# rosielab/emojivoice

Measured on AMD Instinct MI355X. Metric: audio_seconds_per_second, higher is better.
Workload: dtype f32 (deep layers: operand = two block-scaled fp16 pieces, product = 3 fp16 products on the fp16 MFMA, f32 accumulate); 1 GPU; config2: batch 64 x 516-frame (5.99 s) utterances per GPU, 10 Euler steps + HiFi-GAN V1, 22.05 kHz; global_batch=64, frames=516, ode_steps=10, parallelism=dp1, collective=none, batch_pipeline=cfm(i+1) || hifigan(i) on two streams, 2 pipeline(s) in flight

## Files before the change

### emojivoice_amd/_lib.py

```python
from __future__ import annotations

import ctypes as C
import os
import subprocess
from typing import Dict, Optional

import numpy as np
import torch

_HERE = os.path.dirname(os.path.abspath(__file__))
LIB_PATH = os.environ.get("EV_LIB_PATH") or os.path.join(_HERE, "lib", "libemojivoice_hip.so")
CSRC = os.path.join(_HERE, "csrc")
SOURCES = [os.path.join(CSRC, n) for n in ("ev_engine.hip", "ev_kernels.h", "ev_analysis_kernels.h", "ev_analysis.h")] \
    + [os.path.join(os.path.dirname(_HERE), "include", "emojivoice.h")]

EXPORTS = [
    "ev_abi_version", "ev_create", "ev_destroy", "ev_last_error", "ev_load_estimator", "ev_load_vocoder", "ev_load_vocoder_cfg", "ev_load_text_encoder", "ev_text_encoder",
    "ev_text_encoder_status", "ev_stft_magnitude", "ev_denoise", "ev_align", "ev_dbg_conv_bench",
    "ev_workspace_bytes", "ev_cfm_decode", "ev_estimator", "ev_hifigan", "ev_profile_enable", "ev_profile_read", "ev_profile_read_split", "ev_dbg_last_cfg", "ev_set_arithmetic", "ev_get_arithmetic",
    "ev_op_conv1d", "ev_op_groupnorm_mish", "ev_op_groupnorm_mish2", "ev_op_conv_groupnorm", "ev_op_layernorm", "ev_op_split_pieces", "ev_op_attention", "ev_op_ln_mlp", "ev_set_mrf_streams_max",
    "ev_cfm_decode2", "ev_reserve", "ev_alloc_count", "ev_dbg_sk_stats", "ev_op_attn_out", "ev_dbg_set_amax", "ev_dbg_set_attn_h16", "ev_dbg_set_chain", "ev_dbg_sk_taken",
    "ev_load_mel_basis", "ev_mel_spectrogram",
    "ev_maximum_path", "ev_log_prior", "ev_mas_align",
    "ev_estimator_rows", "ev_cfm_loss",
    "ev_load_resampler", "ev_resample", "ev_mel_stats",
    "ev_trim_bounds", "ev_trim_apply",
    "ev_pitch_yin", "ev_dtw",
    "ev_loudness",
    "ev_pyin_observe", "ev_pyin_decode",
    "ev_op_attention2", "ev_op_attn_out2",
    "ev_load_stoi", "ev_stoi",
    "ev_load_stft_dist", "ev_stft_dist",
    "ev_load_voice_quality", "ev_voice_quality",
    "ev_load_formants", "ev_formants",
    "ev_perturbation",
    "ev_load_harmonics", "ev_harmonics",
    "ev_functionals",
    "ev_load_auditory", "ev_auditory",
]


class EvLibraryError(RuntimeError):
    pass


class ev_tensor_index(C.Structure):
    _fields_ = [("name", C.c_char_p), ("offset", C.c_uint64), ("ndim", C.c_int32), ("shape", C.c_int64 * 4)]


class ev_model_dims(C.Structure):
    _fields_ = [("n_feats", C.c_int32), ("spk_emb_dim", C.c_int32), ("channels", C.c_int32), ("heads", C.c_int32),
                ("head_dim", C.c_int32)]


# ... 93 lines not shown
    lib.ev_trim_apply.argtypes = [vp, vp, vp, vp, f32, i32, i32, vp, i32, vp, vp]
    lib.ev_pitch_yin.argtypes = [vp, vp, vp, i32, i32, i32, i32, i32, i32, f32, vp, vp, vp, vp]
    lib.ev_dtw.argtypes = [vp, vp, vp, vp, vp, i32, i32, i32, i32, i32, vp, vp, vp, vp]
    lib.ev_loudness.argtypes = [vp, vp, vp, i32, i32, i32, vp, C.c_double, vp, vp, vp, vp, vp]
    f64 = C.c_double
    lib.ev_pyin_observe.argtypes = [vp, vp, vp, i32, i32, i32, i32, i32, i32, f64, f64, i32, i32, vp, i32, f64, f64, vp, vp, vp]
    lib.ev_pyin_decode.argtypes = [vp, vp, vp, vp, i32, i32, i32, i32, i32, vp, vp, f64, f64, vp, vp, vp, vp]
    lib.ev_load_stoi.argtypes = [vp, vp, vp, vp, i32, i32, i32, i32, i32]
    lib.ev_stoi.argtypes = [vp, vp, vp, vp, i32, i32, C.c_double, C.c_double, vp, vp, vp, vp, vp, vp]
    lib.ev_load_stft_dist.argtypes = [vp, vp, vp, i32, i32, i32]
    lib.ev_stft_dist.argtypes = [vp, vp, vp, vp, i32, i32, C.c_double, vp, vp, vp, vp]
    lib.ev_load_voice_quality.argtypes = [vp, vp, vp, i32, i32, i32, vp, vp, i32, i32, i32, vp, C.c_double]
    lib.ev_voice_quality.argtypes = [vp, vp, vp, i32, i32, C.c_double, vp, vp, vp, vp]
    lib.ev_load_formants.argtypes = [vp, vp, i32, i32, i32, C.c_double, C.c_double, C.c_double, i32]
    lib.ev_formants.argtypes = [vp, vp, vp, i32, i32, C.c_double, vp, vp, vp, vp]
    lib.ev_perturbation.argtypes = [vp, vp, vp, i32, i32, i32, vp, i32, i32, C.c_double, C.c_double, C.c_double, vp, vp, vp, vp]
    lib.ev_load_harmonics.argtypes = [vp, vp, vp, i32, i32, i32, C.c_double, i32, C.c_double, C.c_double, C.c_double]
    lib.ev_harmonics.argtypes = [vp, vp, vp, i32, i32, vp, vp, vp, i32, C.c_double, vp, vp, vp, vp]
    lib.ev_functionals.argtypes = [vp, vp, vp, vp, i32, i32, i32, vp, i32, vp, vp, vp]
    lib.ev_load_auditory.argtypes = [vp, vp, vp, i32, i32, i32, vp, i32, vp, vp, i32, i32, i32, C.c_double]
    lib.ev_auditory.argtypes = [vp, vp, vp, i32, i32, C.c_double, vp, vp, vp, vp, vp]
    lib.ev_maximum_path.argtypes = [vp, vp, vp, vp, i32, i32, i32, vp, vp, vp]
    lib.ev_log_prior.argtypes = [vp, vp, vp, i32, i32, i32, vp, vp]
    lib.ev_mas_align.argtypes = [vp, vp, vp, vp, vp, i32, i32, i32, vp, vp, vp, vp, vp]
    lib.ev_profile_enable.argtypes = [vp, i32]
    lib.ev_profile_read.argtypes = [vp, C.POINTER(C.c_double), C.POINTER(C.c_double), C.POINTER(C.c_int64), i32]
    lib.ev_profile_read_split.argtypes = [vp, C.POINTER(C.c_double), C.POINTER(C.c_double), C.POINTER(C.c_int64)]
    lib.ev_dbg_last_cfg.argtypes = [vp]
    lib.ev_set_arithmetic.argtypes = [vp, i32]
    lib.ev_get_arithmetic.argtypes = [vp]
    lib.ev_dbg_set_amax.argtypes = [vp, i32]
    lib.ev_dbg_set_attn_h16.argtypes = [vp, i32]
    lib.ev_dbg_set_chain.argtypes = [vp, i32]
    lib.ev_dbg_sk_taken.argtypes = [vp]
    lib.ev_dbg_sk_taken.restype = C.c_int64
    lib.ev_op_conv1d.argtypes = [vp, vp, vp, vp, i32, i32, i32, i32, i32, i32, i32, i32, i32, f32, vp, vp]
    lib.ev_op_groupnorm_mish.argtypes = [vp, vp, vp, vp, vp, i32, i32, i32, i32, vp, vp]
    lib.ev_op_groupnorm_mish2.argtypes = [vp, vp, vp, vp, vp, i32, i32, i32, i32, i32, vp, i32, vp, vp, vp]
    lib.ev_op_conv_groupnorm.argtypes = [vp, vp, vp, vp, i32, i32, i32, vp, vp, vp, i32, vp, vp, vp, vp, vp, C.POINTER(C.c_int), vp]
    lib.ev_op_layernorm.argtypes = [vp, vp, vp, vp, i32, i32, vp, vp]
    lib.ev_op_split_pieces.argtypes = [vp, vp, i32, vp, vp]
    lib.ev_op_attention.argtypes = [vp, vp, vp, i32, i32, i32, vp, vp]
    lib.ev_op_attn_out.argtypes = [vp, vp, vp, i32, i32, vp, vp, vp, vp]
    lib.ev_op_attention2.argtypes = [vp, vp, vp, i32, i32, i32, i32, i32, i32, vp, C.POINTER(C.c_int), vp]
    lib.ev_op_attn_out2.argtypes = [vp, vp, vp, i32, i32, i32, i32, vp, vp, f32, f32, f32, vp, C.POINTER(C.c_int), vp]
    lib.ev_op_ln_mlp.argtypes = [vp, vp, vp, vp, vp, vp, vp, vp, vp, vp, vp, i32, i32, i32, vp, vp]
    for n in EXPORTS:
        getattr(lib, n)
    _lib = lib
    return lib


def _stream_ptr() -> int:
    return int(torch.cuda.current_stream().cuda_stream)


def _ptr(t):
    return None if t is None else t.data_ptr()


class Engine:

    def __init__(self, device: int = 0, spk_emb_dim: int = 64, heads: int = 2):
        if not torch.cuda.is_available():
            raise EvLibraryError("no ROCm GPU visible: the EmojiVoice hot path has no CPU fallback")
        self.lib = load_library()
# ... 630 lines not shown
        assert F == 80
        wav = torch.empty((B, 1, T * 256), dtype=torch.float32, device=mel.device)
        per_utt = (T + 2 * self.voc_pad0) * self.voc_frame_bytes
        bmax = max(1, int((2**32 - 2**20) // per_utt))
        for b0 in range(0, B, bmax):
            b1 = min(B, b0 + bmax)
            self._check(self.lib.ev_hifigan(self.h, mel[b0:b1].data_ptr(), b1 - b0, T, wav[b0:b1].data_ptr(), _stream_ptr()), "ev_hifigan")
        return wav

    def workspace_bytes(self, B: int, Tp: int, Tv: int) -> int:
        return int(self.lib.ev_workspace_bytes(self.h, B, Tp, Tv))

    def profile_enable(self, on: bool):
        self._check(self.lib.ev_profile_enable(self.h, int(on)), "ev_profile_enable")

    def op_split_pieces(self, x):
        x = self._f32(x).reshape(-1)
        out = torch.empty((3, x.numel()), dtype=torch.float32, device=x.device)
        self._check(self.lib.ev_op_split_pieces(self.h, x.data_ptr(), x.numel(), out.data_ptr(), _stream_ptr()), "ev_op_split_pieces")
        return out

    def set_arithmetic(self, bf16_products: int):
        self._check(self.lib.ev_set_arithmetic(self.h, int(bf16_products)), "ev_set_arithmetic")

    def set_amax(self, on: bool) -> None:
        self._check(self.lib.ev_dbg_set_amax(self.h, int(bool(on))), "ev_dbg_set_amax")

    def set_attn_h16(self, on: bool) -> None:
        self._check(self.lib.ev_dbg_set_attn_h16(self.h, int(bool(on))), "ev_dbg_set_attn_h16")

    def set_chain(self, on: bool) -> None:
        self._check(self.lib.ev_dbg_set_chain(self.h, int(bool(on))), "ev_dbg_set_chain")

    def arithmetic(self) -> int:
        return int(self.lib.ev_get_arithmetic(self.h))

    def last_cfg(self) -> int:
        return int(self.lib.ev_dbg_last_cfg(self.h))

    def profile_read_split(self):
        ms, fl, n = C.c_double(), C.c_double(), C.c_int64()
        self._check(self.lib.ev_profile_read_split(self.h, C.byref(ms), C.byref(fl), C.byref(n)), "ev_profile_read_split")
        return ms.value, fl.value, n.value

    def profile_read(self, reset: bool = True):
        ms, fl, n = C.c_double(), C.c_double(), C.c_int64()
        self._check(self.lib.ev_profile_read(self.h, C.byref(ms), C.byref(fl), C.byref(n), int(reset)), "ev_profile_read")
        return ms.value, fl.value, n.value

    def op_conv1d(self, x, w, bias, dilation=1, transposed=False, stride=1, padding=0, pre_lrelu_slope=-1.0):
        x = self._f32(x)
        B, Cin, T = x.shape
        w = np.ascontiguousarray(w.detach().cpu().float().numpy())
        if transposed:
            Cout, K = w.shape[1], w.shape[2]
            Tout = T * stride
        else:
            Cout, K = w.shape[0], w.shape[2]
            Tout = T // stride
        bp = None
        if bias is not None:
            bnp = np.ascontiguousarray(bias.detach().cpu().float().numpy())
            bp = bnp.ctypes.data_as(C.c_void_p)
        y = torch.empty((B, Cout, Tout), dtype=torch.float32, device=x.device)
        self._check(self.lib.ev_op_conv1d(self.h, x.data_ptr(), w.ctypes.data_as(C.c_void_p), bp, B, Cin, T, Cout, K, dilation,
                                          int(transposed), stride, padding, float(pre_lrelu_slope), y.data_ptr(), _stream_ptr()),
# ... 129 lines not shown
```

### emojivoice_amd/csrc/ev_engine.hip

```cpp
#include "ev_kernels.h"
#include "../../include/emojivoice.h"

#include <math.h>
#include <stdlib.h>
#include <stdarg.h>
#include <stdio.h>
#include <string.h>

#include <algorithm>
#include <atomic>
#include <mutex>
#include <numeric>
#include <string>
#include <unordered_map>
#include <vector>

namespace {

struct HostTensor {
    const float* p = nullptr;
    int ndim = 0;
    int64_t shape[4] = {0, 0, 0, 0};
    int64_t numel() const { int64_t n = 1; for (int i = 0; i < ndim; ++i) n *= shape[i]; return n; }
};
// ... 89 lines not shown
    int device = 0;
    ev_model_dims dims;
    std::string err;
    std::vector<void*> owned;
    EstimatorW est;
    VocoderW voc;
    TextEncW enc;
    DenoiserW dn;
    MelBasisW melb;
    ResamplerW rs;
    StoiW stoi;
    StftDistW stftd;
    VoiceQW voiceq;
    FormantW fmt;
    HarmW harm;
    AudW aud;
    struct Scratch { char* p = nullptr; size_t bytes = 0; hipStream_t last = nullptr; bool last_valid = false; };
    Scratch dn_ws, enc_ws, mas_ws;
    Scratch dtw_ws;
    Scratch stat_ws;
    Scratch trim_ws;
    Scratch loud_ws;
    Scratch stoi_ws;
    Scratch stftd_ws;
    float* zeros = nullptr;
    int max_steps = 64;
    int* bad_ids_host = nullptr; int* bad_ids_dev = nullptr;
    char* ws = nullptr; size_t ws_bytes = 0; size_t ws_used = 0; size_t ws_bytes_last = 0;
    int ws_B = -1, ws_Tp = -1, ws_Tv = -1;
    bool prof = false;
    bool fuse_pairs = true;
    bool fuse_attn = true;
    bool attn_h16 = true;
    bool use_chain = true;
    bool fuse_mlp = true;
    int gn_stats_tiles = 0;
    int fuse_mlp_min_tiles = 96;
    std::vector<hipEvent_t> ev_pool; size_t ev_used = 0;
    hipStream_t ws_stream = nullptr; bool ws_stream_valid = false;
    float* temb_host[2] = {nullptr, nullptr}; size_t temb_cap[2] = {0, 0}; hipEvent_t temb_ev[2] = {nullptr, nullptr}; int temb_slot = 0;
    float* cap_pool = nullptr; size_t cap_stride = 0; int cap_used = 0; int cap_nt[8] = {0};
    struct TprojEntry { int nt; float* d; };
    std::vector<TprojEntry> tproj_cache;
    bool captured = false; int cap_B = 0, cap_Tp = 0;
    int64_t n_allocs = 0;
    double prof_flops = 0; int64_t prof_launches = 0;
    struct ProfRec { int kind, Cin, Cout, ntaps, nrows, cfg, lean; double flops; bool split = false; };
    std::vector<ProfRec> prof_recs;
    hipStream_t stream = nullptr;
    hipStream_t mrf_stream[2] = {nullptr, nullptr};
    hipEvent_t mrf_ev[4] = {nullptr, nullptr, nullptr, nullptr};
    int ncu = 0;
    unsigned* sk_ctrl = nullptr;
    unsigned sk_seq = 0;
    float* sk_part = nullptr;
    int split_terms = 16;
    bool use_amax = true;
    bool amax_emitted = false;
    int n_fp32_only_layers = 0;
    int last_cfg = -1;
    bool sk_balance = true;
    int sk_wgs = 2;
    int sk_spin = 3000;
    int mrf_max_frames = 16384;
    int force_cfg = -1;
    bool lean = true;
// ... 637 lines not shown
    p.X = X; p.ldx = C; p.Cin = C; p.isplit_log2 = 31;
    p.Mpad = Lc.Mpad; p.Kpad = Lc.Kpad;
    p.Y = Y; p.ldy = C; p.Cout = C; p.osplit_log2 = 31; p.mmul = 1;
    p.nrows = g.nrows; p.S = g.S; p.P = g.P; p.T = g.T;
    p.pro_lrelu = 1; p.pro_slope = 0.1f;
    p.scale = 1.f; p.ldr = C; p.accum = e.accum; p.div3 = e.div3; p.act2_lrelu = e.act2_lrelu; p.act2_slope = e.act2_slope;
    p.yold = e.yold; p.ymax_mul = 1; h->amax_emitted = false;
    p.mtiles = 1; p.ntiles = (g.nrows + out_rows - 1) / out_rows;
}
inline void resblock_bounds(ev_handle* h, ConvParams& p, const Epi& e) {
    if (e.ymax && (!e.accum || e.yold) && h->use_amax) { p.ymax = e.ymax; h->amax_emitted = true; }
}

int launch_pair(ev_handle* h, const ConvLayer& L1, const ConvLayer& L2, const float* X, float* Y, int C, const Geom& g, const Epi& e) {
    if (over_4gib(g, C)) return fail(h, "tensor exceeds the 4 GiB buffer-addressing limit: split the batch");
    if (L1.sparse_taps || L2.sparse_taps || L1.Kpad != C || L2.Kpad != C || L1.Kpad != L2.Kpad || L1.Mpad != L2.Mpad || L1.halo_lo != L1.halo_hi ||
        L2.halo_lo != L2.halo_hi || 2 * L2.halo_lo > 16 || !L1.bias || !L2.bias)
        return fail(h, "launch_pair: unsupported layer pair");
    if (C != 32 && C != 64 && C != 128) return fail(h, "launch_pair: C must be 32, 64 or 128");
    PairParams pp;
    memset(&pp, 0, sizeof pp);
    ConvParams& p = pp.c2;
    const int NT = 8192 / C;
    pp.h1 = L1.halo_lo; pp.h2 = L2.halo_lo; pp.mid_slope = 0.1f; pp.out_rows = NT - 2 * pp.h2;
    resblock_params(h, p, L2, X, Y, C, g, e, pp.out_rows);
    p.W = L2.W; p.bias = L2.bias; p.ntaps = L2.ntaps; p.taplist = L2.taplist[0];
    p.R = X;
    pp.W1 = L1.W; pp.W1x = L1.Wx; p.Wx = L2.Wx; pp.W1h = L1.Wh; pp.w1h_scale = L1.wh_scale; p.Wh = L2.Wh; p.wh_scale = L2.wh_scale; pp.b1 = L1.bias; pp.taplist1 = L1.taplist[0]; pp.ntaps1 = L1.ntaps;
    if (prof_begin(h)) return 1;
    const int lean = epi_flavour(p, h->lean);
    const int split_terms = h->split_terms;
    const bool split = split_terms > 0 && lean != 0 && L1.Wx && L2.Wx && !(e.force_cfg == 0);
    const bool h16 = split && split_terms == 16 && L1.Wh && L2.Wh;
    const dim3 grid(p.ntiles), block(256);
    dispatch<32, 64, 128>(C, [&](auto CC) {
        constexpr int WM = CC / 32, WN = 4 / WM;
        if (h16) {
            resblock_bounds(h, p, e);
            const size_t smem = std::max((size_t)(NT + EV_HALO) * (4 * C + 16) + 64, (size_t)4 * 32 * 36 * sizeof(float));
            dispatch<1, 3>(lean, [&](auto E) { launch<resblock_pair_h16_kernel<WM, WN, E>>(h->device, grid, block, smem, h->stream, pp); });
        } else if (split) {
            const size_t rsb = 6 * C + 16;
            const size_t xs = (size_t)(NT + ((2 * pp.h1 + 7) & ~7)) * rsb, ys = (size_t)(NT + 16) * rsb, es = (size_t)4 * 32 * 36 * sizeof(float);
            const size_t smem = std::max(xs, std::max(ys, es));
            dispatch<1, 3>(lean, [&](auto E) {
                dispatch<3, 6>(split_terms == 3 ? 3 : 6, [&](auto TT) { launch<resblock_pair_split_kernel<WM, WN, E, TT>>(h->device, grid, block, smem, h->stream, pp); });
            });
        } else {
            const size_t xs = (size_t)(NT + ((2 * pp.h1 + 7) & ~7)) * EV_LDK, ys = (size_t)(C / 32) * (NT + 16) * EV_LDK, es = (size_t)4 * 32 * 36;
            const size_t smem = std::max(xs, std::max(ys, es)) * sizeof(float);
            dispatch<0, 1, 3>(lean, [&](auto E) { launch<resblock_pair_kernel<WM, WN, E>>(h->device, grid, block, smem, h->stream, pp); });
        }
    });
    HIPCHK(h, hipGetLastError());
    const int code = (h16 ? 160 : split ? 140 : 100) + L2.ntaps;
    h->last_cfg = code;
    return h->prof ? prof_end(h, {1, C, C, L1.ntaps, g.nrows, code, lean, 2.0 * (L1.macs_per_row + L2.macs_per_row) * valid_rows(g), split}) : 0;
}

inline int chain_halo(const ConvLayer* L1, const ConvLayer* L2) { int hs = 0; for (int m = 0; m < 3; ++m) hs += L1[m].halo_lo + L2[m].halo_lo; return hs; }
inline bool chain_ok(const ev_handle* h, const ConvLayer* L1, const ConvLayer* L2, int C) {
    if (!h->use_chain || h->split_terms != 16 || (C != 32 && C != 64)) return false;
    int hb = 0;
    for (int m = 0; m < 3; ++m) {
        const ConvLayer &a = L1[m], &b = L2[m];
        if (!a.Wh || !b.Wh || !a.bias || !b.bias || a.sparse_taps || b.sparse_taps || a.Kpad != C || b.Kpad != C || a.Mpad != b.Mpad || a.Mpad != L1[0].Mpad ||
            a.halo_lo != a.halo_hi || b.halo_lo != b.halo_hi || a.ntaps != L1[0].ntaps || b.ntaps != L2[0].ntaps || a.ntaps > 64 || b.ntaps > 64) return false;
        hb = std::max(hb, std::max(a.halo_lo, b.halo_lo));
    }
    const int NT = C == 32 ? 256 : 128, hs = chain_halo(L1, L2);
    return hs <= 12 && 2 * hb <= EV_HALO && NT - 2 * hs >= NT / 2;
}
int launch_chain(ev_handle* h, const ConvLayer* L1, const ConvLayer* L2, const float* X, float* Y, int C, const Geom& g, const Epi& e) {
    if (over_4gib(g, C)) return fail(h, "tensor exceeds the 4 GiB buffer-addressing limit: split the batch");
    ChainParams cp;
    memset(&cp, 0, sizeof cp);
    ConvParams& p = cp.c2;
    int hb = 0;
    double macs = 0;
    for (int m = 0; m < 3; ++m) {
        cp.W1h[m] = L1[m].Wh; cp.W2h[m] = L2[m].Wh; cp.w1_scale[m] = L1[m].wh_scale; cp.w2_scale[m] = L2[m].wh_scale;
        cp.b1[m] = L1[m].bias; cp.b2[m] = L2[m].bias; cp.tl1[m] = L1[m].taplist[0]; cp.tl2[m] = L2[m].taplist[0];
        hb = std::max(hb, std::max(L1[m].halo_lo, L2[m].halo_lo));
        macs += L1[m].macs_per_row + L2[m].macs_per_row;
    }
    cp.ntaps1 = L1[0].ntaps; cp.ntaps2 = L2[0].ntaps; cp.hb = hb; cp.halo = chain_halo(L1, L2); cp.mid_slope = 0.1f;
    const int NT = 8192 / C;
    cp.out_rows = NT - 2 * cp.halo;
// ... 1811 lines not shown
            }
        }
    }
    if (conv_ms) *conv_ms = ms;
    if (conv_flops) *conv_flops = h->prof_flops;
    if (conv_launches) *conv_launches = h->prof_launches;
    if (reset) { h->ev_used = 0; h->prof_flops = 0; h->prof_launches = 0; h->prof_recs.clear(); }
    return 0;
}

int ev_dbg_last_cfg(ev_handle* h) { return h ? h->last_cfg : -1; }

int ev_set_arithmetic(ev_handle* h, int bf16_products) {
    if (!h) return 1;
    if (bf16_products != 0 && bf16_products != 3 && bf16_products != 6 && bf16_products != 9 && bf16_products != 16)
        return fail(h, "ev_set_arithmetic: 0, 3, 6, 9 or 16, got %d", bf16_products);
    h->split_terms = bf16_products;
    return 0;
}
int ev_get_arithmetic(ev_handle* h) { return h ? h->split_terms : -1; }

int ev_dbg_set_amax(ev_handle* h, int on) {
    if (!h) return 1;
    h->use_amax = on != 0;
    return 0;
}

int ev_dbg_set_chain(ev_handle* h, int on) {
    if (!h) return 1;
    h->use_chain = on != 0;
    return 0;
}

int ev_dbg_set_attn_h16(ev_handle* h, int on) {
    if (!h) return 1;
    h->attn_h16 = on != 0;
    return 0;
}

int ev_profile_read_split(ev_handle* h, double* ms_out, double* flops_out, int64_t* launches_out) {
    if (!h) return 1;
    HIPCHK(h, hipStreamSynchronize(h->stream));
    double ms = 0, fl = 0;
    int64_t n = 0;
    if (h->prof_recs.size() * 2 == h->ev_used)
        for (size_t i = 0; i < h->prof_recs.size(); ++i) {
            const auto& r = h->prof_recs[i];
            if (!r.split) continue;
            float t = 0;
            HIPCHK(h, hipEventElapsedTime(&t, h->ev_pool[2 * i], h->ev_pool[2 * i + 1]));
            ms += t; fl += r.flops; n += 1;
        }
    if (ms_out) *ms_out = ms;
    if (flops_out) *flops_out = fl;
    if (launches_out) *launches_out = n;
    return 0;
}

int ev_dbg_conv_bench(ev_handle* h, int Cin, int Cout, int K, int dil, int B, int T, int P, int iters, int dbg, int cfg, float* ms_out) {
    const int stagger = (dbg & 64) ? 0 : -1;
    const bool planar = (dbg & 32) != 0;
    const bool no_res = (dbg & 128) != 0;
    const bool no_pro = (dbg & 512) != 0;
    dbg &= ~(64 | 32 | 128 | 512);
    if (enter(h)) return 1;
    h->stream = nullptr;
// ... 384 lines not shown
```

### emojivoice_amd/csrc/ev_kernels.h

```cpp
#pragma once
#include <hip/hip_runtime.h>
#include <stdint.h>
#include <type_traits>

typedef float f32x16 __attribute__((ext_vector_type(16)));
typedef float f32x4 __attribute__((ext_vector_type(4)));
typedef int i32x4 __attribute__((ext_vector_type(4)));

#define EV_MAX_TAPS 16
#define EV_BK 32
#define EV_LDK 36
#define EV_WROWS 128
#define EV_SK_MAXF4(TW) ((TW) == 4 ? (64 + 64) * 8 * 8 : 16 * 512)
#define EV_HALO 64

enum { ACT_NONE = 0, ACT_LRELU = 1, ACT_TANH = 2, ACT_SILU = 3, ACT_MISH = 4, ACT_SNAKE = 5 };

struct SkCtl {
    unsigned* ctrl;
    unsigned* flags;
    float* part;
    int part_floats;
    int q, r;
    int spin_limit;
// ... 2381 lines not shown
    {
#pragma unroll
        for (int j = 0; j < TN; ++j) {
            const int r = wn * (TN * 32) + j * 32 + li;
            const int n = g0 + r;
            const int t = (n >= 0 && n < p.nrows) ? (n % p.S) - p.P : -1;
            const float inside = (t >= 0 && t < p.T) ? 1.f : 0.f;
#pragma unroll
            for (int g = 0; g < 4; ++g) {
                f32x4 v;
#pragma unroll
                for (int e = 0; e < 4; ++e) v[e] = ev_lrelu(acc[0][j][4 * g + e], pp.mid_slope) * inside;
                *(f32x4*)(Ys + (wm * YROWS + r + pp.h2) * EV_LDK + 8 * g + 4 * lh) = v;
            }
        }
        if (tid < 2 * pp.h2 * 8 * NCH) {
            const int chn = tid / (2 * pp.h2 * 8), rem = tid % (2 * pp.h2 * 8);
            const int br = rem / 8, c4 = (rem % 8) * 4;
            const int row = br < pp.h2 ? br : NT + br;
            f32x4 z = {0.f, 0.f, 0.f, 0.f};
            *(f32x4*)(Ys + (chn * YROWS + row) * EV_LDK + c4) = z;
        }
    }
    ev_lds_barrier();

    phase(p.W, p.taplist, p.ntaps, LEAN ? p.bias : nullptr, [&](int ch) -> const float* {
        return Ys + (ch * YROWS + wn * (TN * 32) + li + pp.h2) * EV_LDK + 4 * lh;
    });

    if constexpr (LEAN != 0) conv_epilogue_lean<TM, TN, LEAN>(p, acc, smem + wave * (32 * (TM * 32 + 4)), wm * 32, g0 + wn * (TN * 32), lane, n0, n0 + pp.out_rows);
    else conv_epilogue<TM, TN, false>(p, acc, smem + wave * (32 * (TM * 32 + 4)), wm * 32, g0 + wn * (TN * 32), lane, n0, n0 + pp.out_rows);
}

template <int WAVES_M, int WAVES_N, class PIPE>
struct EvResblockCore {
    static constexpr int TM = 1, TN = 2;
    static constexpr int C = 32 * WAVES_M;
    static constexpr int NT = WAVES_N * TN * 32;
    static constexpr int PIECES = PIPE::PIECES;
    static constexpr unsigned KGB = PIPE::KG_BYTES;
    static constexpr int RSB = PIECES * 2 * C + 16;
    static constexpr int NS = C / 16, H = NS / 2;
    static_assert(WAVES_M * WAVES_N == 4, "4 waves per workgroup");

    char* Xb;
    float* red;
    int tid, lane, wave, wm, wn, li, lh;
    unsigned wlane, wbase;
    f32x16 acc[TM][TN];
    f32x4 A0[PIECES][TM], A1[PIECES][TM], A2[PIECES][TM], A3[PIECES][TM], B0[PIECES][TN], B1[PIECES][TN];

    __device__ __forceinline__ EvResblockCore(char* tile, float* maxima, int Kpad) : Xb(tile), red(maxima) {
        tid = threadIdx.x; lane = tid & 63; wave = __builtin_amdgcn_readfirstlane(tid >> 6);
        wm = wave / WAVES_N; wn = wave % WAVES_N;
        li = lane & 31; lh = lane >> 5;
        wlane = (unsigned)lane * 16u;
        wbase = (unsigned)(wm * (Kpad >> 4)) * KGB;
    }
    __device__ __forceinline__ int row0() const { return wn * (TN * 32); }
    __device__ __forceinline__ const char* bbase(int halo) const { return Xb + (row0() + li + halo) * RSB + 16 * lh; }
    __device__ __forceinline__ bool row_inside(const ConvParams& p, int g0, int j) const {
        const int n = g0 + row0() + j * 32 + li;
        const int t = (n >= 0 && n < p.nrows) ? (n % p.S) - p.P : -1;
        return t >= 0 && t < p.T;
    }

    __device__ __forceinline__ void ldAp(const __amdgpu_buffer_rsrc_t& rW, f32x4 (&dst)[PIECES][TM], unsigned aoff) {
#pragma unroll
        for (int pc = 0; pc < PIECES; ++pc) dst[pc][0] = ev_bload4(rW, wlane, aoff + (unsigned)(pc * 1024));
    }
    __device__ __forceinline__ void ldB(f32x4 (&dst)[PIECES][TN], const char* brow, int slab) {
#pragma unroll
        for (int pc = 0; pc < PIECES; ++pc)
#pragma unroll
            for (int j = 0; j < TN; ++j) dst[pc][j] = *(const f32x4*)(brow + j * 32 * RSB + pc * (2 * C) + slab * 32);
    }
    __device__ __forceinline__ unsigned g_off(int2 tlv, int g, int ngroups) const {
        const int gg = g < ngroups ? g : 0;
        return PIPE::tap_off((unsigned)__builtin_amdgcn_readlane(tlv.x, gg / H)) + wbase + (unsigned)(2 * (gg % H)) * KGB;
    }
    __device__ __forceinline__ int g_row(int2 tlv, int g, int ngroups) const {
        const int gg = g < ngroups ? g : 0;
        return __builtin_amdgcn_readlane(tlv.y, gg / H);
    }
    __device__ __forceinline__ void acc_init(const float* binit, float unit) {
        f32x4 bq[4];
#pragma unroll
        for (int g = 0; g < 4; ++g) bq[g] = *(const f32x4*)(binit + wm * 32 + 8 * g + 4 * lh) * unit;
#pragma unroll
        for (int b = 0; b < TN; ++b)
#pragma unroll
            for (int r = 0; r < 16; ++r) acc[0][b][r] = bq[r >> 2][r & 3];
    }
    __device__ __forceinline__ void ring_fill(const __amdgpu_buffer_rsrc_t& rW, int2 tlv, int ngroups) {
        const unsigned o0 = g_off(tlv, 0, ngroups), o1 = g_off(tlv, 1, ngroups);
        ldAp(rW, A0, o0); ldAp(rW, A1, o0 + KGB); ldAp(rW, A2, o1); ldAp(rW, A3, o1 + KGB);
    }
    __device__ __forceinline__ void group(const __amdgpu_buffer_rsrc_t& rW, int2 tlv, int ngroups, const char* brow0,
                                          f32x4 (&Aa)[PIECES][TM], f32x4 (&Ab)[PIECES][TM], int g) {
        const char* brow = brow0 + g_row(tlv, g, ngroups) * RSB;
        const char* nbrow = brow0 + g_row(tlv, g + 1, ngroups) * RSB;
        const int s0 = 2 * (g % H), ns0 = 2 * ((g + 1) % H);
        const unsigned nap = g_off(tlv, g + 2, ngroups);
        ldB(B1, brow, s0 + 1);
        __builtin_amdgcn_sched_barrier(0);
        PIPE::template mma<TM, TN>(acc, Aa, B0);
        __builtin_amdgcn_sched_barrier(0);
        ldAp(rW, Aa, nap);
        ldB(B0, nbrow, ns0);
        __builtin_amdgcn_sched_barrier(0);
        PIPE::template mma<TM, TN>(acc, Ab, B1);
        __builtin_amdgcn_sched_barrier(0);
        ldAp(rW, Ab, nap + KGB);
    }
    __device__ __forceinline__ void kloop(const __amdgpu_buffer_rsrc_t& rW, int2 tlv, int ngroups, const char* brow0) {
        ldB(B0, brow0 + g_row(tlv, 0, ngroups) * RSB, 0);
        int g = 0;
        for (; g + 1 < ngroups; g += 2) { group(rW, tlv, ngroups, brow0, A0, A1, g); group(rW, tlv, ngroups, brow0, A2, A3, g + 1); }
        if (g < ngroups) group(rW, tlv, ngroups, brow0, A0, A1, g);
    }
    template <int ROW16>
    __device__ __forceinline__ void zero_border_rows(int hb) {
        for (int i = tid; i < 2 * hb * ROW16; i += 256) {
            const int br = i / ROW16, c16 = i % ROW16;
            const int row = br < hb ? br : NT + br;
            uint4 z = {0u, 0u, 0u, 0u};
            *(uint4*)(Xb + row * RSB + c16 * 16) = z;
        }
    }

    __device__ __forceinline__ float hand_over(f32x16 (&v)[TN], int slot, int row_halo) {
        float mx = 0.f;
#pragma unroll
        for (int j = 0; j < TN; ++j)
#pragma unroll
            for (int r = 0; r < 16; r += 2) mx = fmaxf(mx, fmaxf(fabsf(v[j][r]), fabsf(v[j][r + 1])));
        float tmx = evh_wg_max(red, slot, wave, lane, mx);
        if (!evh_is_finite(tmx)) {
            mx = 0.f;
#pragma unroll
            for (int j = 0; j < TN; ++j)
#pragma unroll
                for (int r = 0; r < 16; ++r) { const float a = fabsf(v[j][r]); mx = fmaxf(mx, evh_is_finite(a) ? a : 0.f); }
            tmx = evh_wg_max(red, 8 + slot, wave, lane, mx);
        }
        const float sc = evh_scale_for(tmx);
#pragma unroll
        for (int j = 0; j < TN; ++j) {
            const int r = row0() + j * 32 + li;
#pragma unroll
            for (int g = 0; g < 4; ++g) {
                const f32x4 w = {v[j][4 * g] * sc, v[j][4 * g + 1] * sc, v[j][4 * g + 2] * sc, v[j][4 * g + 3] * sc};
                uint2 q0v, q1v;
                evh_split4(w, q0v, q1v);
                char* dst = Xb + (r + row_halo) * RSB + (wm * 32 + 8 * g + 4 * lh) * 2;
                *(uint2*)(dst) = q0v; *(uint2*)(dst + 2 * C) = q1v;
            }
        }
        return sc;
    }
    __device__ __forceinline__ float conv_from_acc(int slot, int row_halo, const __amdgpu_buffer_rsrc_t& rW, int2 tlv, int ngroups,
                                                   const float* bias, float w_scale) {
        const float u = w_scale * hand_over(acc[0], slot, row_halo);
        acc_init(bias, u);
        ev_lds_barrier();
        kloop(rW, tlv, ngroups, bbase(row_halo));
        return u;
    }

    __device__ __forceinline__ void running_x_load(const ConvParams& p, int g0, int hb, f32x16 (&xr)[TN], float (&inside)[TN]) {
        const __amdgpu_buffer_rsrc_t rX = ev_rsrc(p.X);
#pragma unroll
        for (int j = 0; j < TN; ++j) {
            const int n = g0 + row0() + j * 32 + li;
            const bool in = n >= 0 && n < p.nrows;
            inside[j] = row_inside(p, g0, j) ? 1.f : 0.f;
            const unsigned ro = (in ? (unsigned)n * (unsigned)p.ldx : 0u) * 4u + (unsigned)(wm * 32 + 4 * lh) * 4u;
#pragma unroll
            for (int q = 0; q < 4; ++q) {
                const f32x4 v = ev_bload4(rX, ro + (unsigned)(8 * q) * 4u, 0);
#pragma unroll
                for (int e = 0; e < 4; ++e) xr[j][4 * q + e] = v[e];
            }
        }
        zero_border_rows<RSB / 16>(hb);
    }
    __device__ __forceinline__ void acc_from_lrelu_x(const f32x16 (&xr)[TN], float slope) {
#pragma unroll
        for (int j = 0; j < TN; ++j)
#pragma unroll
            for (int r = 0; r < 16; ++r) acc[0][j][r] = ev_lrelu(xr[j][r], slope);
    }
    __device__ __forceinline__ void running_x_add(f32x16 (&xr)[TN], const float (&inside)[TN], float u) {
        const float inv = 1.0f / u;
#pragma unroll
        for (int j = 0; j < TN; ++j)
#pragma unroll
            for (int r = 0; r < 16; ++r) xr[j][r] = fmaf(acc[0][j][r], inv, xr[j][r]) * inside[j];
    }
    template <int LEAN>
    __device__ __forceinline__ void running_x_store(const ConvParams& p, EvAmax& am, const f32x16 (&xr)[TN], float* smem, int g0, int n0, int out_rows) {
#pragma unroll
        for (int j = 0; j < TN; ++j) acc[0][j] = xr[j];
        ev_amax_from_acc<TM, TN>(p, am, acc, g0 + row0(), lane);
        conv_epilogue_lean<TM, TN, LEAN>(p, acc, smem + wave * (32 * (TM * 32 + 4)), wm * 32, g0 + row0(), lane, n0, n0 + out_rows);
        ev_amax_emit(p, am, g0 + row0(), TN * 32, lane);
    }
};
// ... 53 lines not shown
        }
    }
    ev_lds_barrier();
    k.kloop(rW1, tlv1, ng1, k.bbase(pp.h1));
    k.ring_fill(rW2, tlv2, ng2);

    ev_lds_barrier();
    {
#pragma unroll
        for (int j = 0; j < TN; ++j) {
            const int r = k.row0() + j * 32 + li;
            const float inside = k.row_inside(p, g0, j) ? 1.f : 0.f;
#pragma unroll
            for (int g = 0; g < 4; ++g) {
                f32x4 v;
#pragma unroll
                for (int e = 0; e < 4; ++e) v[e] = ev_lrelu(k.acc[0][j][4 * g + e], pp.mid_slope) * inside;
                uint2 q0v, q1v, q2v;
                evx_split4(v, q0v, q1v, q2v);
                char* dst = Xb + (r + pp.h2) * RSB + (wm * 32 + 8 * g + 4 * lh) * 2;
                *(uint2*)(dst) = q0v; *(uint2*)(dst + 2 * C) = q1v; *(uint2*)(dst + 4 * C) = q2v;
            }
        }
        k.template zero_border_rows<6 * C / 16>(pp.h2);
    }
    k.acc_init(LEAN ? p.bias : pp.b1, 1.f);
    ev_lds_barrier();

    k.kloop(rW2, tlv2, ng2, k.bbase(pp.h2));

    conv_epilogue_lean<TM, TN, LEAN>(p, k.acc, smem + wave * (32 * (TM * 32 + 4)), wm * 32, g0 + k.row0(), lane, n0, n0 + pp.out_rows);
}

template <int WAVES_M, int WAVES_N, int LEAN>
__global__ __launch_bounds__(256, 2) void resblock_pair_h16_kernel(const PairParams pp) {
    using Core = EvResblockCore<WAVES_M, WAVES_N, EvPipeH16>;
    constexpr int TM = Core::TM, TN = Core::TN, C = Core::C, NT = Core::NT, RSB = Core::RSB, H = Core::H;
    constexpr int TPR = C / 4, RPS = 256 / TPR;
    constexpr int XPASS = (NT + EV_HALO) / RPS;
    const ConvParams& p = pp.c2;
    extern __shared__ __attribute__((aligned(16))) float smem[];

    const int nt = ev_xcd_remap(blockIdx.x, p.ntiles);
    const int n0 = nt * pp.out_rows;
    const int g0 = n0 - pp.h2;
    if (ev_tile_is_padding(p.S, p.P, p.T, p.nrows, n0, pp.out_rows)) return;
    Core k((char*)smem, smem + ((NT + EV_HALO) * RSB) / 4, p.Kpad);
    char* Xb = k.Xb;
    const int tid = k.tid, lane = k.lane, wave = k.wave, wm = k.wm;
    const int srow = tid / TPR, sc4 = (tid % TPR) * 4;
    const int nw0 = g0 + k.row0();
    EvAmax am = ev_amax_begin(p, nw0, TN * 32);
    const __amdgpu_buffer_rsrc_t rX = ev_rsrc(p.X);

    const __amdgpu_buffer_rsrc_t rW1 = ev_rsrc(pp.W1h), rW2 = ev_rsrc(p.Wh);
    const int ng1 = pp.ntaps1 * H, ng2 = p.ntaps * H;
    const int2 tlv1 = (lane < pp.ntaps1) ? pp.taplist1[lane] : make_int2(0, 0);
    const int2 tlv2 = (lane < p.ntaps) ? p.taplist[lane] : make_int2(0, 0);
    k.ring_fill(rW1, tlv1, ng1);
    float sx;
    {
        const int xrows = NT + 2 * pp.h1;
        f32x4 xg[XPASS];
        float mx = 0.f;
#pragma unroll
        for (int q = 0; q < XPASS; ++q) {
            const int r = q * RPS + srow;
            const int gr = g0 - pp.h1 + r;
            xg[q] = ev_bload4(rX, ((r < xrows && gr >= 0 && gr < p.nrows) ? (unsigned)gr * (unsigned)p.ldx : 0u) * 4u + (unsigned)sc4 * 4u, 0);
        }
#pragma unroll
        for (int q = 0; q < XPASS; ++q) mx = fmaxf(mx, evh_absmax4(xg[q]));
        float tmx = evh_wg_max(k.red, 0, wave, lane, mx);
        if (!evh_is_finite(tmx)) {
            mx = 0.f;
#pragma unroll
            for (int q = 0; q < XPASS; ++q) mx = fmaxf(mx, evh_absmax4_finite(xg[q]));
            tmx = evh_wg_max(k.red, 8, wave, lane, mx);
        }
        sx = evh_scale_for(tmx);
        am.rlo = am.rhi = tmx;
#pragma unroll
        for (int q = 0; q < XPASS; ++q) {
            const int r = q * RPS + srow;
            f32x4 v = xg[q];
            v[0] = ev_lrelu(v[0], p.pro_slope); v[1] = ev_lrelu(v[1], p.pro_slope);
            v[2] = ev_lrelu(v[2], p.pro_slope); v[3] = ev_lrelu(v[3], p.pro_slope);
            uint2 q0v, q1v;
            evh_split4(v * sx, q0v, q1v);
            if (r < xrows) {
                char* dst = Xb + r * RSB + sc4 * 2;
                *(uint2*)(dst) = q0v; *(uint2*)(dst + 2 * C) = q1v;
            }
        }
    }
    const float u1 = pp.w1h_scale * sx;
    k.acc_init(pp.b1, u1);
    ev_lds_barrier();
    k.kloop(rW1, tlv1, ng1, k.bbase(pp.h1));
    k.ring_fill(rW2, tlv2, ng2);

    float sy;
    {
        const float inv1 = 1.0f / u1;
#pragma unroll
        for (int j = 0; j < TN; ++j) {
            const float inside = k.row_inside(p, g0, j) ? inv1 : 0.f;
#pragma unroll
            for (int r16 = 0; r16 < 16; ++r16) k.acc[0][j][r16] = ev_lrelu(k.acc[0][j][r16] * inside, pp.mid_slope);
        }
        sy = k.hand_over(k.acc[0], 4, pp.h2);
        k.template zero_border_rows<4 * C / 16>(pp.h2);
    }
    const float u2 = p.wh_scale * sy;
    k.acc_init(LEAN ? p.bias : pp.b1, u2);
    ev_lds_barrier();

    k.kloop(rW2, tlv2, ng2, k.bbase(pp.h2));
    {
        const float inv2 = 1.0f / u2;
#pragma unroll
        for (int j = 0; j < TN; ++j)
#pragma unroll
            for (int r16 = 0; r16 < 16; ++r16) k.acc[0][j][r16] *= inv2;
    }
    ev_amax_from_acc<TM, TN>(p, am, k.acc, nw0, lane);
    conv_epilogue_lean<TM, TN, LEAN>(p, k.acc, smem + wave * (32 * (TM * 32 + 4)), wm * 32, nw0, lane, n0, n0 + pp.out_rows);
    ev_amax_emit(p, am, nw0, TN * 32, lane);
}

struct ChainParams {
    ConvParams c2;
    const void* W1h[3]; const void* W2h[3]; float w1_scale[3], w2_scale[3];
    const float* b1[3]; const float* b2[3];
    const int2* tl1[3]; const int2* tl2[3];
    int ntaps1, ntaps2;
    int hb;
    int halo;
    int out_rows;
    float mid_slope;
};
template <int WAVES_M, int WAVES_N, int LEAN>
__global__ __launch_bounds__(256, 2) void resblock_chain_h16_kernel(const ChainParams cp) {
    using Core = EvResblockCore<WAVES_M, WAVES_N, EvPipeH16>;
    constexpr int TN = Core::TN, C = Core::C, NT = Core::NT, RSB = Core::RSB, H = Core::H;
    static_assert(C == 32 || C == 64, "C = 32 / 64");
    const ConvParams& p = cp.c2;
    extern __shared__ __attribute__((aligned(16))) float smem[];
    const int nt = ev_xcd_remap(blockIdx.x, p.ntiles);
    const int n0 = nt * cp.out_rows;
    const int g0 = n0 - cp.halo;
    if (ev_tile_is_padding(p.S, p.P, p.T, p.nrows, n0, cp.out_rows)) return;
    Core k((char*)smem, smem + ((NT + EV_HALO) * RSB) / 4, p.Kpad);
    const int lane = k.lane;
    EvAmax am = ev_amax_begin(p, g0 + k.row0(), TN * 32);
    f32x16 xr[TN];
    float inside[TN];
    k.running_x_load(p, g0, cp.hb, xr, inside);
    const int ng1 = cp.ntaps1 * H, ng2 = cp.ntaps2 * H;
#pragma unroll 1
    for (int m = 0; m < 3; ++m) {
        const __amdgpu_buffer_rsrc_t rW1 = ev_rsrc(cp.W1h[m]), rW2 = ev_rsrc(cp.W2h[m]);
// ... 2801 lines not shown
```

### include/emojivoice.h

```cpp
#ifndef EMOJIVOICE_H
#define EMOJIVOICE_H

#include <stddef.h>
#include <stdint.h>

#ifdef __cplusplus
extern "C" {
#endif

#define EV_ABI_VERSION 4

typedef struct ev_handle ev_handle;

typedef struct ev_tensor_index {
    const char *name;
    uint64_t offset;
    int32_t ndim;
    int64_t shape[4];
} ev_tensor_index;

typedef struct ev_model_dims {
    int32_t n_feats;
    int32_t spk_emb_dim;
    int32_t channels;
// ... 136 lines not shown
int ev_load_harmonics(ev_handle *h, const double *window , const double *twiddle , int W, int H, int nfft,
                      double sr, int n_harm, double search , double min_spacing , double a3_range );
int ev_harmonics(ev_handle *h, const float *d_x , const int32_t *d_len , int B, int L,
                 const float *d_period ,
                 const double *d_formant , const int32_t *d_fcount , int n_formants,
                 double power_floor, double *d_frame , int32_t *d_count ,
                 double *d_harm , void *stream);

int ev_functionals(ev_handle *h, const double *d_v , const uint8_t *d_mask ,
                   const int32_t *d_len , int B, int K, int F,
                   const double *q , int NQ,
                   double *d_stat , int32_t *d_count , void *stream);

int ev_load_auditory(ev_handle *h, const double *window , const double *twiddle , int W, int H, int nfft,
                     const double *mel_w , int n_mel, const double *eq ,
                     const double *dct , int n_ceps, int k_lo, int k_hi, double compress );
int ev_auditory(ev_handle *h, const float *d_x , const int32_t *d_len , int B, int L, double power_floor,
                double *d_frame , double *d_mfcc , int32_t *d_flags ,
                double *d_bands , void *stream);

int ev_profile_enable(ev_handle *h, int on);
int ev_profile_read(ev_handle *h, double *conv_ms, double *conv_flops, int64_t *conv_launches, int reset);
int ev_profile_read_split(ev_handle *h, double *ms, double *flops, int64_t *launches);
int ev_set_arithmetic(ev_handle *h, int setting);
int ev_get_arithmetic(ev_handle *h);

int ev_dbg_last_cfg(ev_handle *h);

int ev_dbg_conv_bench(ev_handle *h, int Cin, int Cout, int K, int dil, int B, int T, int P, int iters, int dbg, int cfg, float *ms_out);

int ev_dbg_set_amax(ev_handle *h, int on);
int ev_dbg_set_attn_h16(ev_handle *h, int on);
int ev_dbg_set_chain(ev_handle *h, int on);

int ev_dbg_sk_stats(ev_handle *h, uint32_t *out3);
int64_t ev_dbg_sk_taken(ev_handle *h);

int ev_op_conv1d(ev_handle *h, const float *d_x , const float *w ,
                 const float *bias , int B, int Cin, int T, int Cout, int K, int dilation,
                 int transposed, int stride, int padding, float pre_lrelu_slope , float *d_y, void *stream);
int ev_op_groupnorm_mish(ev_handle *h, const float *d_x , const float *d_gamma, const float *d_beta,
                         const int32_t *d_lengths, int B, int C, int T, int groups, float *d_y, void *stream);
int ev_op_groupnorm_mish2(ev_handle *h, const float *d_x , const float *d_gamma, const float *d_beta,
                          const int32_t *d_lengths, int B, int C, int T, int groups, int mode, const float *d_temb,
                          int temb_stride, const float *d_R, float *d_y, void *stream);
int ev_op_conv_groupnorm(ev_handle *h, const float *d_x , const float *w ,
                         const float *bias , int Cin, int T, int K, const float *d_gamma,
                         const float *d_beta, const int32_t *d_lengths , int mode, const float *d_temb, const float *d_R,
                         float *d_conv, float *d_part, float *d_y, int *tiles_out, void *stream);
int ev_op_split_pieces(ev_handle *h, const float *d_x, int n, float *d_pieces, void *stream);
int ev_op_layernorm(ev_handle *h, const float *d_x , const float *d_gamma, const float *d_beta, int rows,
                    int C, float *d_y, void *stream);
int ev_op_ln_mlp(ev_handle *h, const float *d_x, const float *d_ln_g, const float *d_ln_b, const float *w1, const float *b1,
                 const float *d_alpha_exp, const float *d_beta_inv, const float *w2, const float *b2, const float *d_rowmask,
                 int rows, int M1, int mode, float *d_y, void *stream);
int ev_op_attention(ev_handle *h, const float *d_qkv , const int32_t *d_lengths, int B, int T,
                    int heads, float *d_out , void *stream);

int ev_op_attn_out(ev_handle *h, const float *d_qkv, const int32_t *d_lengths, int B, int T, const float *w_out, const float *b_out,
                   float *d_hid, void *stream);

int ev_op_attention2(ev_handle *h, const float *d_qkv, const int32_t *d_lengths, int B, int S, int P, int T, int heads, int no_scratch,
                     float *d_out, int *ran, void *stream);
int ev_op_attn_out2(ev_handle *h, const float *d_qkv, const int32_t *d_lengths, int B, int S, int P, int T, const float *w_out,
                    const float *b_out, float sq, float sk, float sv, float *d_hid, int *ran, void *stream);

// ... 5 lines not shown
```

Before: 4822 audio_s/s.

## Add wide-row resblock pair kernel for 128-channel HiFi-GAN layers

Adds a resblock pair kernel variant where each wave computes two 32-channel tiles (TM=2) for C=128. The 2x2 wave layout doubles the row tile to 128 with a 16-row halo, so halo recompute and weight reloads per output row go down. It is selected only when there are enough tiles (at least 5 workgroups per CU) and the kernel taps are small. The cost is more registers and LDS per workgroup, which may lower occupancy. A debug knob sets the threshold and counts launches.

Result: no change. 4839 audio_s/s, median of 6 (+0.3%).

```diff
diff --git a/emojivoice_amd/_lib.py b/emojivoice_amd/_lib.py
--- a/emojivoice_amd/_lib.py
+++ b/emojivoice_amd/_lib.py
@@ -19,7 +19,7 @@
     "ev_text_encoder_status", "ev_stft_magnitude", "ev_denoise", "ev_align", "ev_dbg_conv_bench",
     "ev_workspace_bytes", "ev_cfm_decode", "ev_estimator", "ev_hifigan", "ev_profile_enable", "ev_profile_read", "ev_profile_read_split", "ev_dbg_last_cfg", "ev_set_arithmetic", "ev_get_arithmetic",
     "ev_op_conv1d", "ev_op_groupnorm_mish", "ev_op_groupnorm_mish2", "ev_op_conv_groupnorm", "ev_op_layernorm", "ev_op_split_pieces", "ev_op_attention", "ev_op_ln_mlp", "ev_set_mrf_streams_max",
-    "ev_cfm_decode2", "ev_reserve", "ev_alloc_count", "ev_dbg_sk_stats", "ev_op_attn_out", "ev_dbg_set_amax", "ev_dbg_set_attn_h16", "ev_dbg_set_chain", "ev_dbg_sk_taken",
+    "ev_cfm_decode2", "ev_reserve", "ev_alloc_count", "ev_dbg_sk_stats", "ev_op_attn_out", "ev_dbg_set_amax", "ev_dbg_set_attn_h16", "ev_dbg_set_chain", "ev_dbg_set_pair_wide", "ev_dbg_sk_taken",
     "ev_load_mel_basis", "ev_mel_spectrogram",
     "ev_maximum_path", "ev_log_prior", "ev_mas_align",
     "ev_estimator_rows", "ev_cfm_loss",
@@ -179,6 +179,8 @@
     lib.ev_dbg_set_amax.argtypes = [vp, i32]
     lib.ev_dbg_set_attn_h16.argtypes = [vp, i32]
     lib.ev_dbg_set_chain.argtypes = [vp, i32]
+    lib.ev_dbg_set_pair_wide.argtypes = [vp, i32]
+    lib.ev_dbg_set_pair_wide.restype = C.c_int64
     lib.ev_dbg_sk_taken.argtypes = [vp]
     lib.ev_dbg_sk_taken.restype = C.c_int64
     lib.ev_op_conv1d.argtypes = [vp, vp, vp, vp, i32, i32, i32, i32, i32, i32, i32, i32, i32, f32, vp, vp]
@@ -875,6 +877,12 @@
     def set_chain(self, on: bool) -> None:
         self._check(self.lib.ev_dbg_set_chain(self.h, int(bool(on))), "ev_dbg_set_chain")
 
+    def set_pair_wide(self, min_wg_per_cu: int = -1) -> int:
+        n = int(self.lib.ev_dbg_set_pair_wide(self.h, int(min_wg_per_cu)))
+        if n < 0:
+            raise EvLibraryError("ev_dbg_set_pair_wide failed")
+        return n
+
     def arithmetic(self) -> int:
         return int(self.lib.ev_get_arithmetic(self.h))
 
diff --git a/emojivoice_amd/csrc/ev_engine.hip b/emojivoice_amd/csrc/ev_engine.hip
--- a/emojivoice_amd/csrc/ev_engine.hip
+++ b/emojivoice_amd/csrc/ev_engine.hip
@@ -145,6 +145,8 @@
     bool fuse_pairs = true;
     bool fuse_attn = true;
     bool attn_h16 = true;
+    int pairw_min_wg = 5;
+    int64_t pairw_launches = 0;
     bool use_chain = true;
     bool fuse_mlp = true;
     int gn_stats_tiles = 0;
@@ -848,8 +850,19 @@
     const int split_terms = h->split_terms;
     const bool split = split_terms > 0 && lean != 0 && L1.Wx && L2.Wx && !(e.force_cfg == 0);
     const bool h16 = split && split_terms == 16 && L1.Wh && L2.Wh;
+    bool wide = false;
+    if (h16 && C == 128 && L1.ntaps <= 3 && L2.ntaps <= 3 && 2 * pp.h1 <= EV_PAIRW_HALO && 2 * pp.h2 <= EV_PAIRW_HALO && h->ncu > 0) {
+        const int out_w = 128 - 2 * pp.h2;
+        const long nt_w = ((long)g.nrows + out_w - 1) / out_w;
+        if (nt_w >= (long)h->pairw_min_wg * h->ncu) { wide = true; pp.out_rows = out_w; p.ntiles = (int)nt_w; }
+    }
     const dim3 grid(p.ntiles), block(256);
-    dispatch<32, 64, 128>(C, [&](auto CC) {
+    if (wide) {
+        resblock_bounds(h, p, e);
+        ++h->pairw_launches;
+        const size_t smem = (size_t)(128 + EV_PAIRW_HALO) * (4 * C + 16) + 64;
+        dispatch<1, 3>(lean, [&](auto E) { launch<resblock_pair_h16w_kernel<2, 2, E>>(h->device, grid, block, smem, h->stream, pp); });
+    } else dispatch<32, 64, 128>(C, [&](auto CC) {
         constexpr int WM = CC / 32, WN = 4 / WM;
         if (h16) {
             resblock_bounds(h, p, e);
@@ -869,7 +882,7 @@
         }
     });
     HIPCHK(h, hipGetLastError());
-    const int code = (h16 ? 160 : split ? 140 : 100) + L2.ntaps;
+    const int code = (wide ? 170 : h16 ? 160 : split ? 140 : 100) + L2.ntaps;
     h->last_cfg = code;
     return h->prof ? prof_end(h, {1, C, C, L1.ntaps, g.nrows, code, lean, 2.0 * (L1.macs_per_row + L2.macs_per_row) * valid_rows(g), split}) : 0;
 }
@@ -2747,6 +2760,12 @@
     return 0;
 }
 
+int64_t ev_dbg_set_pair_wide(ev_handle* h, int min_wg_per_cu) {
+    if (!h) return -1;
+    if (min_wg_per_cu >= 0) h->pairw_min_wg = min_wg_per_cu;
+    return h->pairw_launches;
+}
+
 int ev_dbg_set_attn_h16(ev_handle* h, int on) {
     if (!h) return 1;
     h->attn_h16 = on != 0;
diff --git a/emojivoice_amd/csrc/ev_kernels.h b/emojivoice_amd/csrc/ev_kernels.h
--- a/emojivoice_amd/csrc/ev_kernels.h
+++ b/emojivoice_amd/csrc/ev_kernels.h
@@ -2437,21 +2437,21 @@
     else conv_epilogue<TM, TN, false>(p, acc, smem + wave * (32 * (TM * 32 + 4)), wm * 32, g0 + wn * (TN * 32), lane, n0, n0 + pp.out_rows);
 }
 
-template <int WAVES_M, int WAVES_N, class PIPE>
+template <int WAVES_M, int WAVES_N, class PIPE, int TM_ = 1>
 struct EvResblockCore {
-    static constexpr int TM = 1, TN = 2;
-    static constexpr int C = 32 * WAVES_M;
+    static constexpr int TM = TM_, TN = 2;
+    static constexpr int C = 32 * TM * WAVES_M;
     static constexpr int NT = WAVES_N * TN * 32;
     static constexpr int PIECES = PIPE::PIECES;
     static constexpr unsigned KGB = PIPE::KG_BYTES;
     static constexpr int RSB = PIECES * 2 * C + 16;
     static constexpr int NS = C / 16, H = NS / 2;
-    static_assert(WAVES_M * WAVES_N == 4, "4 waves per workgroup");
+    static_assert(WAVES_M * WAVES_N == 4 && (TM == 1 || TM == 2), "4 waves per workgroup");
 
     char* Xb;
     float* red;
     int tid, lane, wave, wm, wn, li, lh;
-    unsigned wlane, wbase;
+    unsigned wlane, wbase, mstep;
     f32x16 acc[TM][TN];
     f32x4 A0[PIECES][TM], A1[PIECES][TM], A2[PIECES][TM], A3[PIECES][TM], B0[PIECES][TN], B1[PIECES][TN];
 
@@ -2460,8 +2460,10 @@
         wm = wave / WAVES_N; wn = wave % WAVES_N;
         li = lane & 31; lh = lane >> 5;
         wlane = (unsigned)lane * 16u;
-        wbase = (unsigned)(wm * (Kpad >> 4)) * KGB;
-    }
+        wbase = (unsigned)(wm * TM * (Kpad >> 4)) * KGB;
+        mstep = (unsigned)(Kpad >> 4) * KGB;
+    }
+    __device__ __forceinline__ int ch0() const { return wm * (TM * 32); }
     __device__ __forceinline__ int row0() const { return wn * (TN * 32); }
     __device__ __forceinline__ const char* bbase(int halo) const { return Xb + (row0() + li + halo) * RSB + 16 * lh; }
     __device__ __forceinline__ bool row_inside(const ConvParams& p, int g0, int j) const {
@@ -2472,7 +2474,9 @@
 
     __device__ __forceinline__ void ldAp(const __amdgpu_buffer_rsrc_t& rW, f32x4 (&dst)[PIECES][TM], unsigned aoff) {
 #pragma unroll
-        for (int pc = 0; pc < PIECES; ++pc) dst[pc][0] = ev_bload4(rW, wlane, aoff + (unsigned)(pc * 1024));
+        for (int pc = 0; pc < PIECES; ++pc)
+#pragma unroll
+            for (int i = 0; i < TM; ++i) dst[pc][i] = ev_bload4(rW, wlane, aoff + (unsigned)i * mstep + (unsigned)(pc * 1024));
     }
     __device__ __forceinline__ void ldB(f32x4 (&dst)[PIECES][TN], const char* brow, int slab) {
 #pragma unroll
@@ -2489,13 +2493,16 @@
         return __builtin_amdgcn_readlane(tlv.y, gg / H);
     }
     __device__ __forceinline__ void acc_init(const float* binit, float unit) {
-        f32x4 bq[4];
-#pragma unroll
-        for (int g = 0; g < 4; ++g) bq[g] = *(const f32x4*)(binit + wm * 32 + 8 * g + 4 * lh) * unit;
-#pragma unroll
-        for (int b = 0; b < TN; ++b)
-#pragma unroll
-            for (int r = 0; r < 16; ++r) acc[0][b][r] = bq[r >> 2][r & 3];
+#pragma unroll
+        for (int i = 0; i < TM; ++i) {
+            f32x4 bq[4];
+#pragma unroll
+            for (int g = 0; g < 4; ++g) bq[g] = *(const f32x4*)(binit + ch0() + i * 32 + 8 * g + 4 * lh) * unit;
+#pragma unroll
+            for (int b = 0; b < TN; ++b)
+#pragma unroll
+                for (int r = 0; r < 16; ++r) acc[i][b][r] = bq[r >> 2][r & 3];
+        }
     }
     __device__ __forceinline__ void ring_fill(const __amdgpu_buffer_rsrc_t& rW, int2 tlv, int ngroups) {
         const unsigned o0 = g_off(tlv, 0, ngroups), o1 = g_off(tlv, 1, ngroups);
@@ -2534,39 +2541,45 @@
         }
     }
 
-    __device__ __forceinline__ float hand_over(f32x16 (&v)[TN], int slot, int row_halo) {
+    __device__ __forceinline__ float hand_over(f32x16 (&v)[TM][TN], int slot, int row_halo) {
         float mx = 0.f;
 #pragma unroll
-        for (int j = 0; j < TN; ++j)
-#pragma unroll
-            for (int r = 0; r < 16; r += 2) mx = fmaxf(mx, fmaxf(fabsf(v[j][r]), fabsf(v[j][r + 1])));
+        for (int i = 0; i < TM; ++i)
+#pragma unroll
+            for (int j = 0; j < TN; ++j)
+#pragma unroll
+                for (int r = 0; r < 16; r += 2) mx = fmaxf(mx, fmaxf(fabsf(v[i][j][r]), fabsf(v[i][j][r + 1])));
         float tmx = evh_wg_max(red, slot, wave, lane, mx);
         if (!evh_is_finite(tmx)) {
             mx = 0.f;
 #pragma unroll
-            for (int j = 0; j < TN; ++j)
-#pragma unroll
-                for (int r = 0; r < 16; ++r) { const float a = fabsf(v[j][r]); mx = fmaxf(mx, evh_is_finite(a) ? a : 0.f); }
+            for (int i = 0; i < TM; ++i)
+#pragma unroll
+                for (int j = 0; j < TN; ++j)
+#pragma unroll
+                    for (int r = 0; r < 16; ++r) { const float a = fabsf(v[i][j][r]); mx = fmaxf(mx, evh_is_finite(a) ? a : 0.f); }
             tmx = evh_wg_max(red, 8 + slot, wave, lane, mx);
         }
         const float sc = evh_scale_for(tmx);
 #pragma unroll
-        for (int j = 0; j < TN; ++j) {
-            const int r = row0() + j * 32 + li;
-#pragma unroll
-            for (int g = 0; g < 4; ++g) {
-                const f32x4 w = {v[j][4 * g] * sc, v[j][4 * g + 1] * sc, v[j][4 * g + 2] * sc, v[j][4 * g + 3] * sc};
-                uint2 q0v, q1v;
-                evh_split4(w, q0v, q1v);
-                char* dst = Xb + (r + row_halo) * RSB + (wm * 32 + 8 * g + 4 * lh) * 2;
-                *(uint2*)(dst) = q0v; *(uint2*)(dst + 2 * C) = q1v;
-            }
-        }
+        for (int i = 0; i < TM; ++i)
+#pragma unroll
+            for (int j = 0; j < TN; ++j) {
+                const int r = row0() + j * 32 + li;
+#pragma unroll
+                for (int g = 0; g < 4; ++g) {
+                    const f32x4 w = {v[i][j][4 * g] * sc, v[i][j][4 * g + 1] * sc, v[i][j][4 * g + 2] * sc, v[i][j][4 * g + 3] * sc};
+                    uint2 q0v, q1v;
+                    evh_split4(w, q0v, q1v);
+                    char* dst = Xb + (r + row_halo) * RSB + (ch0() + i * 32 + 8 * g + 4 * lh) * 2;
+                    *(uint2*)(dst) = q0v; *(uint2*)(dst + 2 * C) = q1v;
+                }
+            }
         return sc;
     }
     __device__ __forceinline__ float conv_from_acc(int slot, int row_halo, const __amdgpu_buffer_rsrc_t& rW, int2 tlv, int ngroups,
                                                    const float* bias, float w_scale) {
-        const float u = w_scale * hand_over(acc[0], slot, row_halo);
+        const float u = w_scale * hand_over(acc, slot, row_halo);
         acc_init(bias, u);
         ev_lds_barrier();
         kloop(rW, tlv, ngroups, bbase(row_halo));
@@ -2579,6 +2592,7 @@
         for (int j = 0; j < TN; ++j) {
             const int n = g0 + row0() + j * 32 + li;
             const bool in = n >= 0 && n < p.nrows;
+            static_assert(TM == 1, "the running x is one 32-channel tile per wave");
             inside[j] = row_inside(p, g0, j) ? 1.f : 0.f;
             const unsigned ro = (in ? (unsigned)n * (unsigned)p.ldx : 0u) * 4u + (unsigned)(wm * 32 + 4 * lh) * 4u;
 #pragma unroll
@@ -2698,12 +2712,15 @@
     conv_epilogue_lean<TM, TN, LEAN>(p, k.acc, smem + wave * (32 * (TM * 32 + 4)), wm * 32, g0 + k.row0(), lane, n0, n0 + pp.out_rows);
 }
 
-template <int WAVES_M, int WAVES_N, int LEAN>
-__global__ __launch_bounds__(256, 2) void resblock_pair_h16_kernel(const PairParams pp) {
-    using Core = EvResblockCore<WAVES_M, WAVES_N, EvPipeH16>;
+#define EV_PAIRW_HALO 16
+template <int WAVES_M, int WAVES_N, int LEAN, int TM_>
+__device__ __forceinline__ void resblock_pair_h16_body(const PairParams& pp) {
+    using Core = EvResblockCore<WAVES_M, WAVES_N, EvPipeH16, TM_>;
     constexpr int TM = Core::TM, TN = Core::TN, C = Core::C, NT = Core::NT, RSB = Core::RSB, H = Core::H;
     constexpr int TPR = C / 4, RPS = 256 / TPR;
-    constexpr int XPASS = (NT + EV_HALO) / RPS;
+    constexpr int XH = TM == 1 ? EV_HALO : EV_PAIRW_HALO;
+    constexpr int XPASS = (NT + XH) / RPS;
+    static_assert((NT + XH) % RPS == 0, "whole staging passes");
     const ConvParams& p = pp.c2;
     extern __shared__ __attribute__((aligned(16))) float smem[];
 
@@ -2711,9 +2728,9 @@
     const int n0 = nt * pp.out_rows;
     const int g0 = n0 - pp.h2;
     if (ev_tile_is_padding(p.S, p.P, p.T, p.nrows, n0, pp.out_rows)) return;
-    Core k((char*)smem, smem + ((NT + EV_HALO) * RSB) / 4, p.Kpad);
+    Core k((char*)smem, smem + ((NT + XH) * RSB) / 4, p.Kpad);
     char* Xb = k.Xb;
-    const int tid = k.tid, lane = k.lane, wave = k.wave, wm = k.wm;
+    const int tid = k.tid, lane = k.lane, wave = k.wave;
     const int srow = tid / TPR, sc4 = (tid % TPR) * 4;
     const int nw0 = g0 + k.row0();
     EvAmax am = ev_amax_begin(p, nw0, TN * 32);
@@ -2773,9 +2790,11 @@
         for (int j = 0; j < TN; ++j) {
             const float inside = k.row_inside(p, g0, j) ? inv1 : 0.f;
 #pragma unroll
-            for (int r16 = 0; r16 < 16; ++r16) k.acc[0][j][r16] = ev_lrelu(k.acc[0][j][r16] * inside, pp.mid_slope);
-        }
-        sy = k.hand_over(k.acc[0], 4, pp.h2);
+            for (int i = 0; i < TM; ++i)
+#pragma unroll
+                for (int r16 = 0; r16 < 16; ++r16) k.acc[i][j][r16] = ev_lrelu(k.acc[i][j][r16] * inside, pp.mid_slope);
+        }
+        sy = k.hand_over(k.acc, 4, pp.h2);
         k.template zero_border_rows<4 * C / 16>(pp.h2);
     }
     const float u2 = p.wh_scale * sy;
@@ -2786,14 +2805,20 @@
     {
         const float inv2 = 1.0f / u2;
 #pragma unroll
-        for (int j = 0; j < TN; ++j)
-#pragma unroll
-            for (int r16 = 0; r16 < 16; ++r16) k.acc[0][j][r16] *= inv2;
+        for (int i = 0; i < TM; ++i)
+#pragma unroll
+            for (int j = 0; j < TN; ++j)
+#pragma unroll
+                for (int r16 = 0; r16 < 16; ++r16) k.acc[i][j][r16] *= inv2;
     }
     ev_amax_from_acc<TM, TN>(p, am, k.acc, nw0, lane);
-    conv_epilogue_lean<TM, TN, LEAN>(p, k.acc, smem + wave * (32 * (TM * 32 + 4)), wm * 32, nw0, lane, n0, n0 + pp.out_rows);
+    conv_epilogue_lean<TM, TN, LEAN>(p, k.acc, smem + wave * (32 * (TM * 32 + 4)), k.ch0(), nw0, lane, n0, n0 + pp.out_rows);
     ev_amax_emit(p, am, nw0, TN * 32, lane);
 }
+template <int WAVES_M, int WAVES_N, int LEAN>
+__global__ __launch_bounds__(256, 2) void resblock_pair_h16_kernel(const PairParams pp) { resblock_pair_h16_body<WAVES_M, WAVES_N, LEAN, 1>(pp); }
+template <int WAVES_M, int WAVES_N, int LEAN>
+__global__ __launch_bounds__(256, 2) void resblock_pair_h16w_kernel(const PairParams pp) { resblock_pair_h16_body<WAVES_M, WAVES_N, LEAN, 2>(pp); }
 
 struct ChainParams {
     ConvParams c2;
diff --git a/include/emojivoice.h b/include/emojivoice.h
--- a/include/emojivoice.h
+++ b/include/emojivoice.h
@@ -192,6 +192,7 @@
 int ev_dbg_set_amax(ev_handle *h, int on);
 int ev_dbg_set_attn_h16(ev_handle *h, int on);
 int ev_dbg_set_chain(ev_handle *h, int on);
+int64_t ev_dbg_set_pair_wide(ev_handle *h, int min_wg_per_cu);
 
 int ev_dbg_sk_stats(ev_handle *h, uint32_t *out3);
 int64_t ev_dbg_sk_taken(ev_handle *h);
```
